# nerfstudio-project/nerfstudio

Hardware: AMD Instinct MI355X
Metric: training rays/sec (4096 rays x 48 samples per GPU) (higher is better)
Workload: dtype f32

## Files before the change

include/nsamd.h:

```cpp
#ifndef NSAMD_H
#define NSAMD_H

#include <stdint.h>

#ifdef __cplusplus
extern "C" {
#endif

typedef void* nsamd_stream_t;

typedef enum nsamd_status {
  NSAMD_OK = 0,
  NSAMD_ERR_INVALID_ARG = -1,
  NSAMD_ERR_UNSUPPORTED = -2,
  NSAMD_ERR_LAUNCH = -3,
  NSAMD_ERR_NO_DEVICE = -4
} nsamd_status;

#define NSAMD_MAX_LEVELS 32

typedef struct nsamd_grid {
  int32_t num_levels;
  int32_t log2_table_size;
  float scalings[NSAMD_MAX_LEVELS];
// ... 66 lines not shown
  int32_t in_dim; int32_t hidden;
  float average_init_density;
} nsamd_density_mlp;

int nsamd_density_mlp_fwd(const float* enc, const float* selector, int64_t M, nsamd_density_mlp mlp,
                          float* density, float* pre, nsamd_stream_t stream);

int nsamd_density_field_fwd(nsamd_points pts, int64_t M, int transform, nsamd_aabb aabb, const float* table,
                            nsamd_grid grid, nsamd_density_mlp mlp, float* enc, float* selector, float* density,
                            float* pre, nsamd_stream_t stream);

int nsamd_density_mlp_bwd(const float* enc, const float* selector, const float* pre, const float* ddensity,
                          int64_t M, nsamd_density_mlp mlp, float* denc, float* dW0, float* db0, float* dW1,
                          float* db1, float* workspace, int64_t workspace_floats, nsamd_stream_t stream);

int nsamd_density_mlp_bwd_gated(const float* enc, const float* selector, const float* pre, const float* ddensity,
                                int64_t M, nsamd_density_mlp mlp, float* denc, float* dW0, float* db0, float* dW1,
                                float* db1, float* workspace, int64_t workspace_floats, const uint32_t* gate,
                                const uint8_t* ray_mask, int32_t samples_per_ray, nsamd_stream_t stream);

typedef struct nsamd_field_mlp {
  const float* base_W0; const float* base_b0;
  const float* base_W1; const float* base_b1;
  const float* head_W0; const float* head_b0;
  const float* head_W1; const float* head_b1;
  const float* head_W2; const float* head_b2;
  const float* appearance;
  int32_t num_images;
  float average_init_density;
  const float* ray_terms;
  const float* ray_inputs;
  float* saved_hb;
  const float* saved_rgb;
} nsamd_field_mlp;

int nsamd_field_ray_terms(const float* directions, const int64_t* camera_indices, const float* appearance_const,
                          int64_t num_rays, nsamd_field_mlp mlp, float* ray_terms, float* ray_inputs,
                          nsamd_stream_t stream);

int nsamd_field_mlp_fwd(const float* enc, const float* selector, const float* directions,
                        const int64_t* camera_indices, const float* appearance_const, int64_t dir_group, int64_t M,
                        nsamd_field_mlp mlp, float* density, float* rgb, nsamd_stream_t stream);

typedef struct nsamd_field_mlp_grads {
  float* base_W0; float* base_b0; float* base_W1; float* base_b1;
  float* head_W0; float* head_b0; float* head_W1; float* head_b1; float* head_W2; float* head_b2;
  float* appearance;
} nsamd_field_mlp_grads;

int nsamd_field_mlp_bwd(const float* enc, const float* selector, const float* directions,
                        const int64_t* camera_indices, const float* appearance_const, int64_t dir_group, int64_t M,
                        nsamd_field_mlp mlp, const float* ddensity, const float* drgb, float* denc,
                        nsamd_field_mlp_grads grads, float* workspace, int64_t workspace_floats,
                        nsamd_stream_t stream);

int64_t nsamd_field_mlp_bwd_scatter_workspace(nsamd_grid grid, int64_t M, int64_t* state_words);
int nsamd_field_mlp_bwd_scatter(nsamd_points pts, int transform, nsamd_aabb aabb, nsamd_grid grid, const float* enc,
                                const float* selector, const float* directions, const int64_t* camera_indices,
                                const float* appearance_const, int64_t dir_group, int64_t M, nsamd_field_mlp mlp,
                                const float* ddensity, const float* drgb, float* denc, nsamd_field_mlp_grads grads,
                                float* workspace, int64_t workspace_floats, float* dtable, float* scatter_workspace,
                                int64_t scatter_workspace_floats, nsamd_stream_t stream);
int nsamd_field_mlp_bwd_scatter_phase(nsamd_points pts, int transform, nsamd_aabb aabb, nsamd_grid grid, const float* enc,
                                      const float* selector, const float* directions, const int64_t* camera_indices,
                                      const float* appearance_const, int64_t dir_group, int64_t M, nsamd_field_mlp mlp,
                                      const float* ddensity, const float* drgb, float* denc, nsamd_field_mlp_grads grads,
// ... 246 lines not shown
```

nerfstudio_amd/_native.py:

```python
from __future__ import annotations

import ctypes as C
import os
from typing import Optional

import torch

_HERE = os.path.dirname(os.path.abspath(__file__))
LIB_PATH = os.path.join(_HERE, "libnsamd.so")

MAX_LEVELS = 32
XFORM_NONE, XFORM_CONTRACT, XFORM_AABB = 0, 1, 2
BG_NONE, BG_LAST_SAMPLE, BG_CONSTANT = 0, 1, 2

vp = C.c_void_p
i64 = C.c_int64
i32 = C.c_int32
f32 = C.c_float


class Grid(C.Structure):
    _fields_ = [("num_levels", i32), ("log2_table_size", i32), ("scalings", f32 * MAX_LEVELS)]


class Points(C.Structure):
    _fields_ = [("positions", vp), ("origins", vp), ("directions", vp), ("t_bins", vp), ("samples_per_ray", i32)]


class Aabb(C.Structure):
    _fields_ = [("lo", f32 * 3), ("hi", f32 * 3)]


class DensityMlp(C.Structure):
    _fields_ = [("W0", vp), ("b0", vp), ("W1", vp), ("b1", vp), ("in_dim", i32), ("hidden", i32),
                ("average_init_density", f32)]


class FieldMlp(C.Structure):
    _fields_ = [("base_W0", vp), ("base_b0", vp), ("base_W1", vp), ("base_b1", vp), ("head_W0", vp), ("head_b0", vp),
                ("head_W1", vp), ("head_b1", vp), ("head_W2", vp), ("head_b2", vp), ("appearance", vp),
                ("num_images", i32), ("average_init_density", f32), ("ray_terms", vp), ("ray_inputs", vp),
                ("saved_hb", vp), ("saved_rgb", vp)]


class OccGrid(C.Structure):
    _fields_ = [("binaries", vp), ("levels", i32), ("resolution", i32), ("aabb", f32 * 6), ("coarse", vp)]


class RayGrads(C.Structure):
    _fields_ = [("d_origins", vp * 4), ("d_directions", vp * 4), ("count", i32)]


class FieldMlpGrads(C.Structure):
    _fields_ = [("base_W0", vp), ("base_b0", vp), ("base_W1", vp), ("base_b1", vp), ("head_W0", vp), ("head_b0", vp),
                ("head_W1", vp), ("head_b1", vp), ("head_W2", vp), ("head_b2", vp), ("appearance", vp)]


class ProposalLevelBwd(C.Structure):
    _fields_ = [("num_rays", i64), ("samples_per_ray", i32),
                ("t_bins", vp), ("density", vp), ("dweights", vp), ("ddensity", vp), ("gate", vp), ("ray_mask", vp),
                ("enc", vp), ("selector", vp), ("pre", vp), ("mlp", DensityMlp), ("denc", vp),
                ("dW0", vp), ("db0", vp), ("dW1", vp), ("db1", vp), ("mlp_workspace", vp), ("mlp_workspace_floats", i64),
                ("origins", vp), ("directions", vp), ("transform", C.c_int), ("aabb", Aabb), ("table", vp), ("grid", Grid),
                ("dtable", vp), ("scatter_workspace", vp), ("scatter_workspace_floats", i64)]


_SIGNATURES = {
    "nsamd_hashgrid_encode_fwd": [Points, i64, C.c_int, Aabb, vp, Grid, vp, i64, i64, vp, vp],
    "nsamd_hashgrid_encode_bwd": [Points, i64, C.c_int, Aabb, vp, Grid, vp, i64, i64, vp, vp, vp, i64, vp],
    "nsamd_hashgrid_encode_bwd_set": [Points, i64, C.c_int, Aabb, vp, Grid, vp, i64, i64, vp, vp, vp, i64, vp],
    "nsamd_hashgrid_encode_bwd_rays": [Points, i64, C.c_int, Aabb, vp, Grid, vp, i64, i64, vp, vp, C.c_int, vp],
    "nsamd_hashgrid_encode_bwd_gated": [Points, i64, C.c_int, Aabb, vp, Grid, vp, i64, i64, vp, vp, i64, vp, vp, vp],
    "nsamd_hashgrid_encode_bwd_rays_gated": [Points, i64, C.c_int, Aabb, vp, Grid, vp, i64, i64, vp, vp, C.c_int, vp, vp, vp],
    "nsamd_hashgrid_encode_bwd_workspace": [Grid, i64, C.c_int],
    "nsamd_hashgrid_encode_bwd_workspace_state": [Grid, i64],
# ... 254 lines not shown
```

nerfstudio_amd/csrc/field_mlp.hip:

```cpp

#include "common.h"
#include "field_reduce.h"
#include "launch.h"
#include "mfma_chain.h"
#include "scatter.h"
#include "wave.h"

NSAMD_PROBE_DEFINE(field)

namespace nsamd {

constexpr int kWaves = 4;
constexpr int kFieldThreads = 64 * kWaves;
constexpr int kScratchLd = 20;
constexpr int kScratchTile = 64 * kScratchLd;

template <int NT, int KT, int THREADS>
__device__ __forceinline__ void stage_frag_load(float* v, const float* __restrict__ W, int n_real, int k_real, bool head0,
                                                int app_dim) {
  static_assert(THREADS % 256 == 0 && (NT * KT * 256) % THREADS == 0, "whole tiles per pass");
  const int r = threadIdx.x & 3, lane = (threadIdx.x >> 2) & 63;
  const int j = lane & 15, g = lane >> 4;
#pragma unroll
  for (int i = 0; i < NT * KT * 256 / THREADS; ++i) {
// ... 169 lines not shown
    asm volatile("" ::: "memory");
    const TileInputs ti = tile_inputs(tile, lane, M, selector, cams, dir_group);
    FieldActs A;
    load_enc_tile_fwd(enc, M, ti.p, lane, A.enc);
    if (RAYC && rgb != nullptr) {
      const float* c = mlp.ray_terms + ti.ray * 64 + 4 * (lane >> 4);
#pragma unroll
      for (int n = 0; n < 4; ++n) A.ha[n] = *reinterpret_cast<const v4f*>(c + 16 * n);
    }
    PROBE_STAMP(WAVES, 2 + 4 * probe_it);
    field_forward_tile<RAYC>(wf, bias, directions, app_table, app_const, dir_group, M, app_dim, ti, lane, A, 3 + 4 * probe_it,
                             rgb == nullptr);
    PROBE_STAMP(WAVES, 4 + 4 * probe_it);
    if (rgb != nullptr && mlp.saved_hb != nullptr && ti.live) {
#pragma unroll
      for (int t = 0; t < 4; ++t) *reinterpret_cast<v4f*>(mlp.saved_hb + ((tile * 4 + t) * 64 + lane) * 4) = A.hb[t];
    }
    if (lane < 16 && ti.live) {
      density[ti.p] = mlp.average_init_density * expf(A.o16[0][0]) * ti.sel;
      if (rgb != nullptr) {
        float* o = rgb + 3 * ti.p;
#pragma unroll
        for (int c = 0; c < 3; ++c) o[c] = 1.0f / (1.0f + expf(-A.rgbp[0][c]));
      }
    }
    PROBE_STAMP(WAVES, 5 + 4 * probe_it);
    ++probe_it;
  }
  PROBE_STAMP(WAVES, 63);
}

__global__ __launch_bounds__(kFieldThreads) void field_ray_terms_kernel(
    const float* __restrict__ directions, const int64_t* __restrict__ cams, const float* __restrict__ app_const,
    int64_t num_rays, nsamd_field_mlp mlp, int app_dim, float* __restrict__ terms, float* __restrict__ inputs) {
  __shared__ __attribute__((aligned(16))) float wf[kFragHead0];
  __shared__ __attribute__((aligned(16))) float bias[64];
  {
    float v[16];
    stage_frag_load<4, 4, kFieldThreads>(v, mlp.head_W0, 64, 31 + app_dim, true, app_dim);
    stage_frag_store<4, 4, kFieldThreads>(wf, v);
    stage_bias<kFieldThreads>(bias, mlp.head_b0, 64, 64);
  }
  __syncthreads();
  const int lane = threadIdx.x & 63, wave = threadIdx.x >> 6;
  const int j = lane & 15, g = lane >> 4;
  const float* app_table = cams ? mlp.appearance : nullptr;
  const int64_t tiles = (num_rays + 15) / 16;
  for (int64_t tile = (int64_t)blockIdx.x * kWaves + wave; tile < tiles; tile += (int64_t)gridDim.x * kWaves) {
    const int64_t ray = tile * 16 + j;
    const bool live = ray < num_rays;
    const int64_t rc = live ? ray : num_rays - 1;
    const float* d = directions + 3 * rc;
    v4f hin[4];
    hin[0] = sh_quad(d[0], d[1], d[2], g);
    if (app_dim > 0) {
      const float* src = (app_table != nullptr) ? app_table + cams[rc] * 32 : app_const;
      hin[2] = *reinterpret_cast<const v4f*>(src + 4 * g);
      hin[3] = *reinterpret_cast<const v4f*>(src + 16 + 4 * g);
    } else {
      hin[2] = v4f{0.f, 0.f, 0.f, 0.f};
      hin[3] = v4f{0.f, 0.f, 0.f, 0.f};
    }
    v4f acc[4];
    load_bias<4>(bias, acc, g);
    chain_gemm_tile<4, 4>(wf, 0, hin[0], acc, lane);
    chain_gemm_tile<4, 4>(wf, 2, hin[2], acc, lane);
    chain_gemm_tile<4, 4>(wf, 3, hin[3], acc, lane);
    if (live) {
#pragma unroll
// ... 961 lines not shown

using namespace nsamd;

static int field_app_dim(const nsamd_field_mlp& mlp, const int64_t* cams, const float* app_const, int* app_dim) {
  if (cams != nullptr) NSAMD_REQUIRE(mlp.appearance != nullptr && mlp.num_images > 0);
  *app_dim = (cams != nullptr || app_const != nullptr) ? 32 : 0;
  return NSAMD_OK;
}

static int field_common_checks(const float* enc, const float* directions, int64_t dir_group, int64_t M,
                               const nsamd_field_mlp& mlp, const int64_t* cams, const float* app_const, int* app_dim) {
  NSAMD_REQUIRE(M >= 0 && dir_group >= 1);
  if (M > kMaxFieldPoints) return NSAMD_ERR_UNSUPPORTED;
  NSAMD_REQUIRE(enc && directions);
  NSAMD_REQUIRE(mlp.base_W0 && mlp.base_b0 && mlp.base_W1 && mlp.base_b1 && mlp.head_W0 && mlp.head_b0 &&
                mlp.head_W1 && mlp.head_b1 && mlp.head_W2 && mlp.head_b2);
  return field_app_dim(mlp, cams, app_const, app_dim);
}

static unsigned field_blocks(int64_t tiles, int waves) {
  return (unsigned)min((int64_t)device_cus(), (tiles + waves - 1) / waves);
}

static unsigned field_bwd_blocks(int64_t M) { return field_blocks((M + 15) / 16, kCoopWaves); }

static bool field_ray_terms_apply(const nsamd_field_mlp& mlp, int64_t dir_group, int64_t M) {
  return mlp.ray_terms != nullptr && dir_group % 16 == 0 && M % dir_group == 0;
}

extern "C" int nsamd_field_ray_terms(const float* directions, const int64_t* camera_indices, const float* appearance_const,
                                     int64_t num_rays, nsamd_field_mlp mlp, float* ray_terms, float* ray_inputs,
                                     nsamd_stream_t stream) {
  NSAMD_REQUIRE(num_rays >= 0);
  if (num_rays == 0) return NSAMD_OK;
  NSAMD_REQUIRE(directions && ray_terms && mlp.head_W0 && mlp.head_b0);
  int app_dim = 0;
  if (const int st = field_app_dim(mlp, camera_indices, appearance_const, &app_dim)) return st;
  const unsigned blocks = field_blocks((num_rays + 15) / 16, kWaves);
  field_ray_terms_kernel<<<blocks, kFieldThreads, 0, (hipStream_t)stream>>>(directions, camera_indices, appearance_const, num_rays,
                                                                           mlp, app_dim, ray_terms, ray_inputs);
  NSAMD_CHECK_LAUNCH();
  return NSAMD_OK;
}

extern "C" int nsamd_field_mlp_fwd(const float* enc, const float* selector, const float* directions,
                                   const int64_t* camera_indices, const float* appearance_const, int64_t dir_group,
                                   int64_t M, nsamd_field_mlp mlp, float* density, float* rgb,
                                   nsamd_stream_t stream) {
  if (M == 0) return NSAMD_OK;
  int app_dim = 0;
  int st = field_common_checks(enc, directions, dir_group, M, mlp, camera_indices, appearance_const, &app_dim);
  if (st) return st;
  NSAMD_REQUIRE(density != nullptr);
  const size_t lds = sizeof(float) * (kFragTotal + 256);
  const unsigned blocks = field_blocks((M + 15) / 16, 16);
  if (field_ray_terms_apply(mlp, dir_group, M) && rgb != nullptr)
    field_mlp_fwd_kernel<16, true><<<blocks, 1024, lds, (hipStream_t)stream>>>(
        enc, selector, directions, camera_indices, appearance_const, dir_group, M, mlp, app_dim, density, rgb);
  else
    field_mlp_fwd_kernel<16><<<blocks, 1024, lds, (hipStream_t)stream>>>(
        enc, selector, directions, camera_indices, appearance_const, dir_group, M, mlp, app_dim, density, rgb);
  NSAMD_CHECK_LAUNCH();
  return NSAMD_OK;
}

struct FieldBwdCall {
  const float *enc, *selector, *directions;
  const int64_t* cams;
  const float* app_const;
  int64_t dir_group, M;
  nsamd_field_mlp mlp;
  const float *ddensity, *drgb;
  float* denc;
// ... 156 lines not shown
```

nerfstudio_amd/functional.py:

```python
from __future__ import annotations

import ctypes as C
import math
from dataclasses import dataclass
from typing import Optional, Sequence, Tuple

import torch
from torch import Tensor

from . import _native as N


_GRID_CACHE: dict = {}

DIRECT_GRAD = False


def _grad_target(param: Tensor, needed: bool):
    if not needed:
        return None, None
    if DIRECT_GRAD and getattr(param, "grad", None) is not None and param.grad.is_contiguous():
        return param.grad, None
    buf = torch.zeros_like(param)
    return buf, buf
# ... 197 lines not shown
def field_mlp(params: Sequence[Tensor], appearance: Optional[Tensor], average_init_density: float,
              ray_terms: Optional[Tensor] = None, ray_inputs: Optional[Tensor] = None) -> N.FieldMlp:
    fm = N.FieldMlp(*(N.ptr(p) for p in params), N.ptr(appearance), appearance.shape[0] if appearance is not None else 0,
                    float(average_init_density))
    fm.ray_terms, fm.ray_inputs = N.ptr(ray_terms), N.ptr(ray_inputs)
    return fm


def field_mlp_grads(params: Sequence[Tensor], appearance: Optional[Tensor], grad_of) -> N.FieldMlpGrads:
    return N.FieldMlpGrads(*(N.ptr(grad_of(p)) for p in params), N.ptr(grad_of(appearance)) if appearance is not None else None)


def hash_forward(pts: N.Points, M: int, transform: int, box: N.Aabb, table: Tensor, grid: HashGridSpec, enc: Tensor,
                 stride_p: int, stride_k: int, sel: Optional[Tensor]) -> None:
    N.check(N.load().nsamd_hashgrid_encode_fwd(pts, M, transform, box, N.ptr(table), grid.native(), N.ptr(enc), stride_p,
                                               stride_k, N.ptr(sel), N.stream()), "hashgrid_encode_fwd")


def table_scatter(pts: N.Points, M: int, transform: int, box: N.Aabb, table: Tensor, grid: HashGridSpec, denc: Tensor,
                  stride_p: int, stride_k: int, dtable: Optional[Tensor], dpos: Optional[Tensor] = None,
                  write_only: bool = False) -> None:
    lib = N.load()
    ws, ws_n = _scatter_workspace(grid, denc.device, M, write_only=write_only)
    fn = lib.nsamd_hashgrid_encode_bwd_set if write_only else lib.nsamd_hashgrid_encode_bwd
    N.check(fn(pts, M, transform, box, N.ptr(table), grid.native(), N.ptr(denc), stride_p, stride_k, N.ptr(dtable), N.ptr(dpos),
               N.ptr(ws), ws_n, N.stream()), "hashgrid_encode_bwd")


def ray_terms_apply(dir_group: int, M: int) -> bool:
    return dir_group % 16 == 0 and M % dir_group == 0 and M > 0


def ray_terms_launch(dirs: Tensor, cams: Optional[Tensor], app_const: Optional[Tensor], rays: int, mlp: N.FieldMlp,
                     terms: Tensor, inputs: Optional[Tensor]) -> None:
    N.check(N.load().nsamd_field_ray_terms(N.ptr(dirs), N.ptr(cams), N.ptr(app_const), rays, mlp, N.ptr(terms), N.ptr(inputs),
                                           N.stream()), "field_ray_terms")


def field_forward(table: Tensor, grid: HashGridSpec, transform: int, box: N.Aabb, pts: N.Points, M: int, enc: Tensor,
                  sel: Tensor, dirs: Tensor, cams: Optional[Tensor], app_const: Optional[Tensor], dir_group: int,
                  mlp: N.FieldMlp, density: Tensor, rgb: Optional[Tensor]) -> None:
    hash_forward(pts, M, transform, box, table, grid, enc, 1, M, sel)
    N.check(N.load().nsamd_field_mlp_fwd(N.ptr(enc), N.ptr(sel), N.ptr(dirs), N.ptr(cams), N.ptr(app_const), dir_group, M, mlp,
                                         N.ptr(density), N.ptr(rgb), N.stream()), "field_mlp_fwd")


def field_backward(table: Tensor, grid: HashGridSpec, transform: int, box: N.Aabb, pts: N.Points, M: int, enc: Tensor,
                   sel: Tensor, dirs: Tensor, cams: Optional[Tensor], app_const: Optional[Tensor], dir_group: int,
                   mlp: N.FieldMlp, ddens: Tensor, drgb: Tensor, denc: Tensor, grads: N.FieldMlpGrads, fws: Tensor,
                   dtable: Optional[Tensor], write_only: bool, fuse: bool = True, keep_denc: bool = False, on_denc=None,
                   fused_launch=None, dpos: Optional[Tensor] = None) -> None:
    lib, st = N.load(), N.stream()
    if fuse and write_only and dpos is None and grid.num_levels == 16:
        sws, sws_n = _producer_scatter_workspace(grid, denc.device, M)
        if sws is not None:
            args = (pts, transform, box, grid.native(), N.ptr(enc), N.ptr(sel), N.ptr(dirs), N.ptr(cams),
                    N.ptr(app_const), dir_group, M, mlp, N.ptr(ddens), N.ptr(drgb), N.ptr(denc) if keep_denc else None, grads,
                    N.ptr(fws), fws.numel(), N.ptr(dtable), N.ptr(sws), sws_n)
            if fused_launch is not None:
                fused_launch(args)
            else:
                N.check(lib.nsamd_field_mlp_bwd_scatter(*args, st), "field_mlp_bwd_scatter")
            return
    N.check(lib.nsamd_field_mlp_bwd(N.ptr(enc), N.ptr(sel), N.ptr(dirs), N.ptr(cams), N.ptr(app_const), dir_group, M, mlp,
                                    N.ptr(ddens), N.ptr(drgb), N.ptr(denc), grads, N.ptr(fws), fws.numel(), st), "field_mlp_bwd")
    if on_denc is not None:
        on_denc()
    if dtable is not None or dpos is not None:
        table_scatter(pts, M, transform, box, table, grid, denc, 1, M, dtable, dpos, write_only=write_only)
# ... 1156 lines not shown
```

nerfstudio_amd/train_step.py:

```python
from __future__ import annotations

import ctypes as C
import os
from typing import Dict, Optional

import torch
from torch import Tensor

from . import _native as N
from . import functional as F
from .nerfacto import NerfactoModel
from .runner_interface import TrainStepRunner
from .utils import profiler


class NerfactoTrainStep(TrainStepRunner):
    def __init__(self, model: NerfactoModel, num_rays: int, device, compute_depths: bool = True,
                 forward_only: bool = False) -> None:
        self.model = model
        self.forward_only = bool(forward_only)
        cfg = model.config
        self.cfg = cfg
        self.n = n = int(num_rays)
        self.counts = (*cfg.num_proposal_samples_per_ray, cfg.num_nerf_samples_per_ray)
# ... 51 lines not shown
        self.d_rgb_s, self.d_dens_main = t(mm, 3), t(mm)
        self._pl_s_bins = N.ptr_array(self.s_bins[: self.n_prop])
        self._pl_weights = N.ptr_array(self.weights[: self.n_prop])
        self._pl_per_ray = N.ptr_array(self.inter_per_ray)
        self._pl_dw = N.ptr_array(self.dw_prop)
        self._pl_S = (C.c_int32 * self.n_prop)(*self.counts[: self.n_prop])
        self.ray_terms_on = F.ray_terms_apply(self.counts[-1], mm)
        self.ray_terms = e(n, 64) if self.ray_terms_on else None
        self.ray_inputs = e(n, 16 + (32 if fld.embedding_appearance is not None else 0)) \
            if (self.ray_terms_on and not forward_only) else None
        self.saved_hb = None if forward_only else torch.zeros(((mm + 15) // 16, 4, 64, 4), **f32)
        self._saved_fresh = False
        self.f_denc = t(*self.f_enc.shape)
        self.p_ddens = [t(*x.shape) for x in self.p_dens]
        self.p_denc = [t(*x.shape) for x in self.p_enc]
        self.field_ws = None if forward_only else F.field_bwd_workspace(device)[0]
        self.density_ws = [] if forward_only else [F.density_bwd_workspace(device, slot=lvl) for lvl in range(self.n_prop)]
        self.gate_proposals = True
        self.prop_gates = torch.zeros(max(self.n_prop, 1) * 4, device=device, dtype=torch.int32)
        self.gates_precleared = False
        self.prop_ray_masks = [torch.zeros(n, device=device, dtype=torch.uint8) for _ in range(self.n_prop)]
        self.fuse_route = os.environ.get("NSAMD_FUSE_ROUTE", "1") == "1"
        self.keep_denc = False
        self.merge_prop_levels = True
        self.loss_vals = torch.zeros(32, **f32)
        self._loss_vals_fresh = False
        self.want_loss_vals = False
        self.pending_select = None
        self.depth = None
        self._depth_buffers = None
        self._slot0 = None
        self._outputs = None
        self.fuse_select = os.environ.get("NSAMD_FUSE_SELECT", "1") == "1"
        self.side_stream = torch.cuda.Stream(device=device)
        self._fork, self._join = torch.cuda.Event(), torch.cuda.Event()
        self._open_branches = []
        self.reduce_stream = torch.cuda.Stream(device=device)
        self._red_fork, self._red_join = torch.cuda.Event(), torch.cuda.Event()
        co = getattr(model, "camera_optimizer", None)
        self.cam_opt = co if (co is not None and co.config.mode != "off") else None
        self.cam_kernels = False
        if self.cam_opt is not None:
            pose = getattr(co, "pose_adjustment", None)
            self.cam_kernels = (os.environ.get("NSAMD_CAMERA_KERNELS", "1") == "1" and pose is not None and pose.is_cuda
                                and pose.dtype == torch.float32 and pose.dim() == 2 and pose.shape[1] == 6
                                and co.config.mode in ("SO3xR3", "SE3")
                                and len(self.counts) + int(want_normals) <= 4
                                and getattr(co, "non_trainable_camera_indices", None) is None)
            self.cam_mode = F.CAMERA_MODES.get(co.config.mode, 0)
            self.raw_origins, self.raw_directions = e(n, 3), e(n, 3)
            self.d_origins = [e(n, 3) for _ in self.counts]
            self.d_directions = [e(n, 3) for _ in self.counts]
            self._corrected = None
            self.camera_reg = torch.zeros((), **f32)
        self.normals = self._normals_buffers(device) if want_normals else None
        self._normals_fresh = False
        self.reg_in_backward = True
        self.cameras_outside = False
        self.grad_lookup = None
        self.main_table_write_only = True
        self.spacing = int(getattr(model.proposal_sampler.initial_sampler, "spacing", 0))
        self.edges = F._linspace("edges", self.counts[0], device)
        self.u_base = [None] + [F._linspace("u", s, device) for s in self.counts[1:]]

    def set_batch(self, origins: Tensor, directions: Tensor, camera_indices: Tensor,
                  target_rgb: Optional[Tensor] = None) -> None:
# ... 134 lines not shown
            self.p_enc[lvl] = torch.empty((self.props[lvl].encoding.get_out_dim(), m), device=dev)
            self.p_sel[lvl] = torch.empty((m,), device=dev)

    def _grad(self, p: Tensor) -> Tensor:
        if self.grad_lookup is not None:
            g = self.grad_lookup.get(id(p))
            if g is not None:
                return g
        assert p.grad is not None and p.grad.is_contiguous(), "parameters need preallocated .grad (use arena.ParamArena)"
        return p.grad

    def _points(self, lvl: int) -> N.Points:
        return N.make_points(None, self.origins, self.directions, self.t_bins[lvl], self.counts[lvl])

    def forward_backward(self, updated: bool, draw_jitter: bool = True) -> None:
        if self.forward_only:
            raise RuntimeError("NerfactoTrainStep(forward_only=True) has no gradient buffers")
        self.forward_and_losses(updated, draw_jitter)
        self.backward_all(updated)

    def proposal_branches(self):
        return [] if self.side_stream is None else [(self.side_stream, self._join, None)]

    def backward_all(self, updated: bool) -> None:
        self.backward_fork(updated)
        self.backward_join(updated)

    def backward_fork(self, updated: bool) -> None:
        branches = self.proposal_branches() if updated else []
        self._open_branches = branches
        if branches:
            main = N.current_stream()
            self._fork.record(main)
            for stream, join, levels in branches:
                stream.wait_event(self._fork)
                with N.on_stream(stream):
                    self.backward_proposals(levels=levels)
                    join.record(stream)
            self.backward_main()
            if self.normals is not None:
                self.normals_backward()
        else:
            self.backward_main()
            if self.normals is not None:
                self.normals_backward()
            if updated:
                self.backward_proposals()

    def backward_join(self, updated: bool) -> None:
        main = N.current_stream()
        for _, join, _ in self._open_branches:
            main.wait_event(join)
        self._open_branches = []
        self.backward_cameras(updated)

    def forward_backward_main(self, updated: bool, draw_jitter: bool = True) -> None:
        self.forward_and_losses(updated, draw_jitter)
        self.backward_main()
        if self.normals is not None:
            self.normals_backward()

    def written_params(self):
        return [self.model.field.mlp_base.encoding.hash_table] if self.main_table_write_only else []

    def forward_and_losses(self, updated: bool, draw_jitter: bool = True) -> None:
        self.apply_camera_corrections()
        self.forward_proposals(draw_jitter, need_enc=updated)
        self.forward_main_and_losses(updated)

    def apply_camera_corrections(self) -> None:
        if self.cam_opt is None:
            return
        if self.cam_kernels:
            F.camera_apply_launch(self.cam_opt.pose_adjustment, self.cam_mode, self.raw_origins, self.raw_directions,
# ... 112 lines not shown
                                  None if self.forward_only else self.p_pre[lvl])
            else:
                ck(fused, "density_field_fwd")
            S2 = self.counts[lvl + 1]
            if per_edge:
                F.weights_launch(self.t_bins[lvl], self.p_dens[lvl], self.weights[lvl])
                if self.compute_depths:
                    F.composite_launch(None, self.weights[lvl], self.t_bins[lvl], N.BG_NONE, None, False, None, None, None,
                                       self.depth_med[lvl], None, None)
                F.pdf_resample_launch(self.s_bins[lvl], self.weights[lvl], self.u_base[lvl + 1], self.jitter_edges[lvl + 1],
                                      self.nears, self.fars, 1.0, self.anneal_dev, 0.01, 1e-5, self.spacing, 1, False, S2,
                                      self.s_bins[lvl + 1], self.t_bins[lvl + 1], None)
                continue
            ck(lib.nsamd_proposal_resample(N.ptr(self.t_bins[lvl]), N.ptr(self.s_bins[lvl]), N.ptr(self.p_dens[lvl]), S,
                                           N.ptr(self.u_base[lvl + 1]), N.ptr(self.jitter[lvl + 1]) if stratified else None,
                                           N.ptr(self.nears),
                                           N.ptr(self.fars), 1.0, N.ptr(self.anneal_dev), 0.01, 1e-5,
                                           1.0 / (2 * (S2 + 1)), self.spacing, n, S2, N.ptr(self.weights[lvl]),
                                           N.ptr(self.depth_med[lvl]) if self.compute_depths else None,
                                           N.ptr(self.s_bins[lvl + 1]), N.ptr(self.t_bins[lvl + 1]), st),
               "proposal_resample")

    def forward_main_and_losses(self, updated: bool, terms_ready: bool = False) -> None:
        self.forward_main(terms_ready)
        self.losses(updated)

    def _field_mlp(self) -> N.FieldMlp:
        fld = self.model.field
        return F.field_mlp(*F.field_params(fld), fld.average_init_density)

    def _cams(self, app_const: Optional[Tensor]) -> Optional[Tensor]:
        return self.camera_indices if (self.model.field.embedding_appearance is not None and app_const is None) else None

    def ray_terms_launch(self, fm: Optional[N.FieldMlp] = None, app_const: Optional[Tensor] = None) -> None:
        F.ray_terms_launch(self.directions, self._cams(app_const), app_const, self.n, fm if fm is not None else self._field_mlp(),
                           self.ray_terms, self.ray_inputs if app_const is None else None)

    @profiler.time_function
    def forward_main(self, terms_ready: bool = False, app_const: Optional[Tensor] = None) -> None:
        L = self.n_prop
        fm = self._field_mlp()
        if self.ray_terms_on:
            if not terms_ready:
                self.ray_terms_launch(fm, app_const)
            fm.ray_terms = N.ptr(self.ray_terms)
            fm.ray_inputs = N.ptr(self.ray_inputs if app_const is None else None)
        self._saved_fresh = self.saved_hb is not None and app_const is None
        if self._saved_fresh:
            fm.saved_hb = N.ptr(self.saved_hb)
        fld = self.model.field
        tbl = fld.mlp_base.encoding
        F.field_forward(tbl.hash_table, tbl.spec, fld._transform, fld._box, self._points(L), self.m_main, self.f_enc, self.f_sel,
                        self.directions, self._cams(app_const), app_const, self.counts[L], fm, self.f_dens, self.f_rgb)
        self._normals_fresh = False

    @profiler.time_function
    def losses(self, updated: bool) -> None:
        lib, st, n, cfg = N.load(), N.stream(), self.n, self.cfg
        ck = N.check
        L = self.n_prop
        S = self.counts[L]
        self._loss_vals_fresh = False
        ck(lib.nsamd_render_train(N.ptr(self.f_rgb), N.ptr(self.f_dens), N.ptr(self.t_bins[L]), n, S, self.bg_mode,
                                  self.bg_vals, N.ptr(self.target), 1.0 / (3 * n), N.ptr(self.weights[L]), N.ptr(self.rgb),
                                  N.ptr(self.acc), N.ptr(self.depth_exp),
                                  N.ptr(self.depth_med[L]) if self.compute_depths else None, N.ptr(self.minmax_ws),
                                  N.ptr(self.sq_err), N.ptr(self.d_rgb_out), N.ptr(self.bg_rays), st), "render_train")
        ck(lib.nsamd_proposal_losses(N.ptr(self.s_bins[L]), N.ptr(self.weights[L]), S, self.n_prop, self._pl_s_bins,
                                     self._pl_weights, self._pl_S, n, float(cfg.interlevel_loss_mult) / (n * S),
# ... 183 lines not shown
```

nerfstudio_amd/trainer.py:

```python
from __future__ import annotations

import os
import sys
from typing import Callable, Dict, NamedTuple, Optional

import torch

from . import _native as N
from .runner_interface import TrainStepRunner

BATCH_SLOTS = 8

_HYPER = {"fields": 0, "proposal_networks": 2, "camera_opt": 6}
_HYPER_ANNEAL, _HYPER_SLOT, _HYPER_FLOATS = 4, 5, 8


class SchedulePlan(NamedTuple):
    dp: bool
    dp_sharded: bool
    dp_fork: bool
    use_graph: bool
    defer: bool
    cam_inside: bool
    cameras_outside: bool
# ... 35 lines not shown
            raise ValueError("HipTrainer: a batch source needs the explicit kernel schedule (use_runner)")
        if runner is not None and not isinstance(runner, TrainStepRunner):
            raise TypeError(f"HipTrainer: the runner must be a runner_interface.TrainStepRunner, got {type(runner).__name__}")
        self.model, self.arena, self.rb, self.batch, self.world = model, arena, ray_bundle, batch, world
        self.pool, self.source = pool, source
        self.slots = int(pool["origins"].shape[0]) if pool is not None else 1
        self.step = self.opt_step = 0
        self.drive_callbacks = drive_callbacks
        self._true_steps = dict(arena.step_counts)
        dev = ray_bundle.origins.device
        self.on_gpu = dev.type == "cuda"
        self.hyper = torch.zeros(_HYPER_FLOATS, device=dev)
        self.hyper_ring = [torch.zeros(_HYPER_FLOATS).pin_memory() if self.on_gpu else torch.zeros(_HYPER_FLOATS) for _ in range(64)]
        self.hyper_ring_np = [h.numpy() for h in self.hyper_ring]
        self.hyper_events = [None] * 64
        self.hyper_slot = 0
        if lr_source is None:
            from .schedulers import ExponentialDecayScheduler, ExponentialDecaySchedulerConfig, nerfacto_schedulers

            sched = nerfacto_schedulers()
            sched["camera_opt"] = ExponentialDecayScheduler(ExponentialDecaySchedulerConfig(lr_final=1e-4, max_steps=5000))
            base = {"fields": arena.lr, "proposal_networks": arena.lr, "camera_opt": 1e-3}
            lr_source = lambda group, it: sched[group].get_lr(max(it, 0), base[group])
        self.lr_source = lr_source
        self.exchange = None
        self.ring_rows = 256
        self.hyper_views = {g: self.hyper[o:o + 2] for g, o in _HYPER.items()}
        self.loss_buf = torch.zeros((), device=dev)
        model.proposal_sampler.anneal_dev = self.hyper[_HYPER_ANNEAL:_HYPER_ANNEAL + 1]
        self.graphs = None
        self._capture_tried = False
        self.defer_scatter = False
        self.opt_parallel = True
        self.draw_jitter = True
        self._pending_main = False
        self.cam_group = "camera_opt" if "camera_opt" in arena.groups else None
        own_runner = runner is None
        if use_runner and own_runner:
            from .train_step import NerfactoTrainStep

            runner = NerfactoTrainStep(model, ray_bundle.origins.shape[0], dev)
        self.runner = r = runner
        defer_env = os.environ.get("NSAMD_DEFER_MAIN_ADAM")
        plan = plan_schedule(runner=r, own_runner=own_runner, world=world, force_dp=force_dp, dp_mode=dp_mode, use_graph=use_graph,
                             on_gpu=self.on_gpu, cam_group=self.cam_group is not None, has_source=source is not None,
                             cameras_outside_switch=os.environ.get("NSAMD_CAMERAS_OUTSIDE", "0") == "1",
                             defer_switch=None if defer_env is None else defer_env == "1")
        (self.dp, self.dp_sharded, self.dp_fork, self.use_graph, self.defer, self.cam_inside, cameras_outside, self.prologue,
         self.prologue_ring, self.source_inside, gates_precleared) = plan
        if r is None:
            return
        r.grad_lookup = arena.grad_lookup()
        r.gates_precleared, r.cameras_outside = gates_precleared, cameras_outside
        r.set_batch(ray_bundle.origins, ray_bundle.directions, ray_bundle.camera_indices, batch["image"])
        r.anneal_dev = self.hyper[_HYPER_ANNEAL:_HYPER_ANNEAL + 1]
        if self.defer:
            self.opt_stream = torch.cuda.Stream(device=dev)
            self._opt_fork, self._opt_join, self._batch_ready = torch.cuda.Event(), torch.cuda.Event(), torch.cuda.Event()
        if self.prologue:
            self.step_counter = torch.zeros(2, device=dev, dtype=torch.int64)
            self.step_counter[1] = int(getattr(model, "step", 0) or 0)
            rank = 0
            if world > 1 and os.environ.get("NSAMD_BENCH_SAME_RAYS") != "1":
                import torch.distributed as dist

                rank = dist.get_rank() if dist.is_available() and dist.is_initialized() else 0
# ... 74 lines not shown
        r = self.runner
        draw = self.draw_jitter
        j = r.jitter if draw else None
        bg = r.bg_rays if (draw and r.bg_rays is not None) else None
        rows_ptr, rows = (self.ring_host.data_ptr(), self.ring_rows) if self.prologue_ring else (None, 0)
        N.check(N.load().nsamd_step_prologue(
            N.ptr(self.step_counter), rows_ptr, rows, N.ptr(self.hyper), N.ptr(j), j.numel() if j is not None else 0,
            N.ptr(bg), bg.numel() if bg is not None else 0, self.rng_seed, N.stream()), "step_prologue")

    def _zero(self, updated, groups=None):
        whole = groups is None
        if groups is None:
            groups = ["fields", "proposal_networks"] if updated else ["fields"]
            if self.cam_inside:
                groups = groups + [self.cam_group]
        self.arena.zero_grad(groups, skip=self.runner.written_params())
        if whole and updated:
            self._clear_gates()

    def _clear_gates(self):
        if self.runner.gates_precleared:
            self.runner.prop_gates.zero_()

    def _stepped(self, updated, pending):
        return ((["fields"] if pending or not self.defer else []) + (["proposal_networks"] if updated else [])
                + ([self.cam_group] if self.cam_inside else []))

    def _body(self, updated, pending):
        r, a = self.runner, self.arena
        assert self.defer or not pending
        beside = pending and self.opt_parallel
        main = N.current_stream() if beside else None
        terms_beside = beside and r.ray_terms_on

        def terms_behind_batch():
            self._batch_ready.record(main)
            self.opt_stream.wait_event(self._batch_ready)
            with N.on_stream(self.opt_stream):
                r.ray_terms_launch()
                self._opt_join.record(self.opt_stream)

        self._step_prologue()
        if beside:
            self._opt_fork.record(main)
            self.opt_stream.wait_event(self._opt_fork)
            with N.on_stream(self.opt_stream):
                a.step(grad_scale=1.0, groups=["fields"], hyper_dev=self.hyper_views)
                self._zero(updated)
                if not terms_beside:
                    self._opt_join.record(self.opt_stream)
        elif pending:
            a.step(grad_scale=1.0, groups=["fields"], hyper_dev=self.hyper_views)
        if not r.cameras_outside:
            self._select_batch()
            r.apply_camera_corrections()
        if not self.defer:
            self._zero(updated)
        r.forward_proposals(self.draw_jitter and not self.prologue, need_enc=updated, after_bins=terms_behind_batch if terms_beside else None)
        if beside:
            main.wait_event(self._opt_join)
        elif self.defer:
            self._zero(updated)
        r.forward_main_and_losses(updated, terms_ready=terms_beside)
        r.backward_all(updated)
        late = self._stepped(updated, pending=False)
        if late:
            a.step(grad_scale=1.0, groups=late, hyper_dev=self.hyper_views)

    def _module_body(self, updated):
        from .cameras.rays import RayBundle

        self._select_batch()
        self.arena.zero_grad()
        m = self.model
        m.proposal_sampler.force_updated = updated
        rb = RayBundle(origins=self.rb.origins, directions=self.rb.directions, pixel_area=self.rb.pixel_area,
                       camera_indices=self.rb.camera_indices)
        out = m(rb)
        metrics = m.get_metrics_dict(out, self.batch)
        loss_dict = m.get_loss_dict(out, self.batch, metrics)
        loss = sum(loss_dict.values())
        loss.backward()
        self.loss_buf.copy_(loss.detach())
        if self.dp:
            self.arena.all_reduce()
        self.arena.step(grad_scale=1.0 / self.world, groups=self._stepped(updated, pending=False), hyper_dev=self.hyper_views)

    def _select_batch(self):
        if self.source is not None:
            if self.source_inside:
                r = self.runner
                co = r.cam_opt is not None
                o, d = (r.raw_origins, r.raw_directions) if co else (r.origins, r.directions)
                self.source.launch(o, d, r.camera_indices, r.target, self.step_counter[1:], -1)
            return
        if self.pool is None:
            return
        from . import functional as F

        p = self.pool
        if self.runner is not None:
            r = self.runner
            co = r.cam_opt is not None
            if not co and r.fuse_select:
                r.pending_select = (N.ptr(self.hyper[_HYPER_SLOT:_HYPER_SLOT + 1]), self.slots, p)
                return
            o, d = (r.raw_origins, r.raw_directions) if co else (r.origins, r.directions)
            c, t = r.camera_indices, r.target
        else:
            o, d, c, t = self.rb.origins, self.rb.directions, self.rb.camera_indices, self.batch["image"]
        F.select_batch_launch(self.hyper[_HYPER_SLOT:_HYPER_SLOT + 1], self.slots, p["origins"], p["directions"], p["cameras"],
                              p["target"], o, d, c, t)

    def _source_batch(self):
        rb, batch = self.source.next_batch()
        self.runner.set_batch(rb.origins, rb.directions, rb.camera_indices.reshape(-1), batch["image"])

    @property
    def _cams_outside(self):
        return self.runner is not None and self.runner.cameras_outside

    def _cameras_before(self):
        self._select_batch()
        self.runner.apply_camera_corrections()

    def _cameras_after(self, updated):
        a, g = self.arena, self.cam_group
        if g is None:
            return
        a.zero_grad([g])
        self.runner.backward_cameras(updated, force=True)
        if self.dp:
            h = a.all_reduce_group(g)
            if h is not None:
                h.wait()
        a.step(grad_scale=1.0 / self.world, groups=[g], hyper_dev=self.hyper_views)

    @property
# ... 164 lines not shown
```

Measured before the change: 6.886 million.

## Compute ray terms from batch pool on optimizer stream and launch main backward first

The ray-terms kernel can now read directions and camera indices straight from the batch pool, using a device-side slot index. This lets it run on the optimizer side stream right after the field step, so it no longer waits on the main stream's batch selection and proposal bins. Separately, the main-chain backward (and the normals backward) is now issued before the proposal backward branches are forked onto side streams. Both changes reorder cross-stream work to shorten the critical path, at the cost of more plumbing and different stream contention.

```diff
diff --git a/include/nsamd.h b/include/nsamd.h
--- a/include/nsamd.h
+++ b/include/nsamd.h
@@ -122,6 +122,8 @@
   const float* ray_inputs;
   float* saved_hb;
   const float* saved_rgb;
+  const float* batch_slot;
+  int32_t batch_slots;
 } nsamd_field_mlp;
 
 int nsamd_field_ray_terms(const float* directions, const int64_t* camera_indices, const float* appearance_const,
diff --git a/nerfstudio_amd/_native.py b/nerfstudio_amd/_native.py
--- a/nerfstudio_amd/_native.py
+++ b/nerfstudio_amd/_native.py
@@ -40,7 +40,7 @@
     _fields_ = [("base_W0", vp), ("base_b0", vp), ("base_W1", vp), ("base_b1", vp), ("head_W0", vp), ("head_b0", vp),
                 ("head_W1", vp), ("head_b1", vp), ("head_W2", vp), ("head_b2", vp), ("appearance", vp),
                 ("num_images", i32), ("average_init_density", f32), ("ray_terms", vp), ("ray_inputs", vp),
-                ("saved_hb", vp), ("saved_rgb", vp)]
+                ("saved_hb", vp), ("saved_rgb", vp), ("batch_slot", vp), ("batch_slots", i32)]
 
 
 class OccGrid(C.Structure):
diff --git a/nerfstudio_amd/csrc/field_mlp.hip b/nerfstudio_amd/csrc/field_mlp.hip
--- a/nerfstudio_amd/csrc/field_mlp.hip
+++ b/nerfstudio_amd/csrc/field_mlp.hip
@@ -225,9 +225,16 @@
 
 __global__ __launch_bounds__(kFieldThreads) void field_ray_terms_kernel(
     const float* __restrict__ directions, const int64_t* __restrict__ cams, const float* __restrict__ app_const,
-    int64_t num_rays, nsamd_field_mlp mlp, int app_dim, float* __restrict__ terms, float* __restrict__ inputs) {
+    int64_t num_rays, nsamd_field_mlp mlp, int app_dim, float* __restrict__ terms, float* __restrict__ inputs,
+    const float* __restrict__ slot_dev, int32_t slots) {
   __shared__ __attribute__((aligned(16))) float wf[kFragHead0];
   __shared__ __attribute__((aligned(16))) float bias[64];
+  if (slot_dev != nullptr) {
+    int32_t slot = (int32_t)slot_dev[0];
+    slot = slot < 0 ? 0 : (slot >= slots ? slots - 1 : slot);
+    directions += (int64_t)slot * 3 * num_rays;
+    if (cams != nullptr) cams += (int64_t)slot * num_rays;
+  }
   {
     float v[16];
     stage_frag_load<4, 4, kFieldThreads>(v, mlp.head_W0, 64, 31 + app_dim, true, app_dim);
@@ -1255,13 +1262,15 @@
                                      int64_t num_rays, nsamd_field_mlp mlp, float* ray_terms, float* ray_inputs,
                                      nsamd_stream_t stream) {
   NSAMD_REQUIRE(num_rays >= 0);
+  NSAMD_REQUIRE(mlp.batch_slot != nullptr ? mlp.batch_slots >= 1 : mlp.batch_slots == 0);
   if (num_rays == 0) return NSAMD_OK;
   NSAMD_REQUIRE(directions && ray_terms && mlp.head_W0 && mlp.head_b0);
   int app_dim = 0;
   if (const int st = field_app_dim(mlp, camera_indices, appearance_const, &app_dim)) return st;
   const unsigned blocks = field_blocks((num_rays + 15) / 16, kWaves);
   field_ray_terms_kernel<<<blocks, kFieldThreads, 0, (hipStream_t)stream>>>(directions, camera_indices, appearance_const, num_rays,
-                                                                           mlp, app_dim, ray_terms, ray_inputs);
+                                                                           mlp, app_dim, ray_terms, ray_inputs, mlp.batch_slot,
+                                                                           mlp.batch_slots);
   NSAMD_CHECK_LAUNCH();
   return NSAMD_OK;
 }
diff --git a/nerfstudio_amd/functional.py b/nerfstudio_amd/functional.py
--- a/nerfstudio_amd/functional.py
+++ b/nerfstudio_amd/functional.py
@@ -253,9 +253,13 @@
 
 
 def ray_terms_launch(dirs: Tensor, cams: Optional[Tensor], app_const: Optional[Tensor], rays: int, mlp: N.FieldMlp,
-                     terms: Tensor, inputs: Optional[Tensor]) -> None:
-    N.check(N.load().nsamd_field_ray_terms(N.ptr(dirs), N.ptr(cams), N.ptr(app_const), rays, mlp, N.ptr(terms), N.ptr(inputs),
-                                           N.stream()), "field_ray_terms")
+                     terms: Tensor, inputs: Optional[Tensor], slot=None, slots: int = 0) -> None:
+    mlp.batch_slot, mlp.batch_slots = slot, slots
+    try:
+        N.check(N.load().nsamd_field_ray_terms(N.ptr(dirs), N.ptr(cams), N.ptr(app_const), rays, mlp, N.ptr(terms),
+                                               N.ptr(inputs), N.stream()), "field_ray_terms")
+    finally:
+        mlp.batch_slot, mlp.batch_slots = None, 0
 
 
 def field_forward(table: Tensor, grid: HashGridSpec, transform: int, box: N.Aabb, pts: N.Points, M: int, enc: Tensor,
diff --git a/nerfstudio_amd/train_step.py b/nerfstudio_amd/train_step.py
--- a/nerfstudio_amd/train_step.py
+++ b/nerfstudio_amd/train_step.py
@@ -107,6 +107,7 @@
         self._slot0 = None
         self._outputs = None
         self.fuse_select = os.environ.get("NSAMD_FUSE_SELECT", "1") == "1"
+        self.main_chain_first = True
         self.side_stream = torch.cuda.Stream(device=device)
         self._fork, self._join = torch.cuda.Event(), torch.cuda.Event()
         self._open_branches = []
@@ -307,14 +308,19 @@
         if branches:
             main = N.current_stream()
             self._fork.record(main)
+            if self.main_chain_first:
+                self.backward_main()
+                if self.normals is not None:
+                    self.normals_backward()
             for stream, join, levels in branches:
                 stream.wait_event(self._fork)
                 with N.on_stream(stream):
                     self.backward_proposals(levels=levels)
                     join.record(stream)
-            self.backward_main()
-            if self.normals is not None:
-                self.normals_backward()
+            if not self.main_chain_first:
+                self.backward_main()
+                if self.normals is not None:
+                    self.normals_backward()
         else:
             self.backward_main()
             if self.normals is not None:
@@ -493,9 +499,16 @@
     def _cams(self, app_const: Optional[Tensor]) -> Optional[Tensor]:
         return self.camera_indices if (self.model.field.embedding_appearance is not None and app_const is None) else None
 
-    def ray_terms_launch(self, fm: Optional[N.FieldMlp] = None, app_const: Optional[Tensor] = None) -> None:
-        F.ray_terms_launch(self.directions, self._cams(app_const), app_const, self.n, fm if fm is not None else self._field_mlp(),
-                           self.ray_terms, self.ray_inputs if app_const is None else None)
+    def ray_terms_launch(self, fm: Optional[N.FieldMlp] = None, app_const: Optional[Tensor] = None, select=None) -> None:
+        fm = fm if fm is not None else self._field_mlp()
+        inputs = self.ray_inputs if app_const is None else None
+        if select is not None:
+            assert self.cam_opt is None
+            slot, slots, pool = select
+            F.ray_terms_launch(pool["directions"], None if self._cams(app_const) is None else pool["cameras"], app_const, self.n,
+                               fm, self.ray_terms, inputs, slot=slot, slots=slots)
+            return
+        F.ray_terms_launch(self.directions, self._cams(app_const), app_const, self.n, fm, self.ray_terms, inputs)
 
     @profiler.time_function
     def forward_main(self, terms_ready: bool = False, app_const: Optional[Tensor] = None) -> None:
diff --git a/nerfstudio_amd/trainer.py b/nerfstudio_amd/trainer.py
--- a/nerfstudio_amd/trainer.py
+++ b/nerfstudio_amd/trainer.py
@@ -91,6 +91,7 @@
         self._capture_tried = False
         self.defer_scatter = False
         self.opt_parallel = True
+        self.terms_from_pool = True
         self.draw_jitter = True
         self._pending_main = False
         self.cam_group = "camera_opt" if "camera_opt" in arena.groups else None
@@ -231,6 +232,8 @@
         beside = pending and self.opt_parallel
         main = N.current_stream() if beside else None
         terms_beside = beside and r.ray_terms_on
+        select = self._pool_select() if (terms_beside and self.terms_from_pool and not r.cameras_outside) else None
+        terms_after_bins = terms_beside and select is None
 
         def terms_behind_batch():
             self._batch_ready.record(main)
@@ -246,7 +249,9 @@
             with N.on_stream(self.opt_stream):
                 a.step(grad_scale=1.0, groups=["fields"], hyper_dev=self.hyper_views)
                 self._zero(updated)
-                if not terms_beside:
+                if select is not None:
+                    r.ray_terms_launch(select=select)
+                if not terms_after_bins:
                     self._opt_join.record(self.opt_stream)
         elif pending:
             a.step(grad_scale=1.0, groups=["fields"], hyper_dev=self.hyper_views)
@@ -255,7 +260,7 @@
             r.apply_camera_corrections()
         if not self.defer:
             self._zero(updated)
-        r.forward_proposals(self.draw_jitter and not self.prologue, need_enc=updated, after_bins=terms_behind_batch if terms_beside else None)
+        r.forward_proposals(self.draw_jitter and not self.prologue, need_enc=updated, after_bins=terms_behind_batch if terms_after_bins else None)
         if beside:
             main.wait_event(self._opt_join)
         elif self.defer:
@@ -285,6 +290,12 @@
             self.arena.all_reduce()
         self.arena.step(grad_scale=1.0 / self.world, groups=self._stepped(updated, pending=False), hyper_dev=self.hyper_views)
 
+    def _pool_select(self):
+        r = self.runner
+        if self.source is not None or self.pool is None or r is None or r.cam_opt is not None or not r.fuse_select:
+            return None
+        return (N.ptr(self.hyper[_HYPER_SLOT:_HYPER_SLOT + 1]), self.slots, self.pool)
+
     def _select_batch(self):
         if self.source is not None:
             if self.source_inside:
@@ -301,8 +312,9 @@
         if self.runner is not None:
             r = self.runner
             co = r.cam_opt is not None
-            if not co and r.fuse_select:
-                r.pending_select = (N.ptr(self.hyper[_HYPER_SLOT:_HYPER_SLOT + 1]), self.slots, p)
+            select = self._pool_select()
+            if select is not None:
+                r.pending_select = select
                 return
             o, d = (r.raw_origins, r.raw_directions) if co else (r.origins, r.directions)
             c, t = r.camera_indices, r.target
```

Result: faster. 7.001 million (median of 6 runs) (+1.7%).
